# Shamir-Lab/Faucet

Hardware: AMD Instinct MI355X
Metric: canonical k-mers/s (load+scan) at k=31, 100bp reads; % HBM roofline (higher is better)
Workload: dtype u64

## Files before the change

### faucet_amd/csrc/fgpu_ctx.h

```cpp
#pragma once
#include <chrono>
#include <hip/hip_runtime.h>
#include <stdint.h>
#include <stdio.h>
#include <string.h>

#include <string>
#include <thread>
#include <vector>

#include "../../include/faucet_gpu.h"
#include <deque>

#include "fgpu_device.h"

#define FGPU_PADW 8
#define FGPU_USUAL_SPAN (1ULL << 26)
#define FGPU_MAX_SPAN (1ULL << 26)

#define FGPU_RANGE_EVENTS 16
#define FGPU_RANGE_MIN (1ULL << 20)

struct DevBuf {
    void*    p = nullptr;
    uint64_t bytes = 0;
};

struct BatchBufs {
    DevBuf codes, bad;
    DevBuf readflag;
    DevBuf pending;
    DevBuf sure;
    DevBuf fail;
    DevBuf same;
    DevBuf valid, pm, ps, ff, fb, cf0, cf1, cb0, cb1, inF, inB;
    DevBuf lk;
    DevBuf cand;
    uint32_t cand_gen = 0;
    DevBuf nF, nB, need;
    DevBuf kh;
    DevBuf cr;
    DevBuf ps_prefix;
    DevBuf pieces;
    DevBuf sF, sB;
    DevBuf piece_read;
    DevBuf stop_off, stop_out;
    const uint64_t* d_offs = nullptr;
    uint64_t seq = 0;
    bool stops_pending = false;
    uint64_t T = 0;
    uint64_t n_words = 0;
    uint64_t n_reads = 0;
    uint64_t n_pieces = 0;
    uint64_t max_piece_span = 0;
    hipEvent_t pure_done = nullptr;
    hipEvent_t range_ev[FGPU_RANGE_EVENTS] = {};
    uint64_t range_first = 0;
    uint64_t range_span = 0;
    uint64_t n_ranges = 0;
    uint64_t ranges_waited = 0;
    hipEvent_t walk_done = nullptr;
    bool walk_pending = false;
    uint32_t planes_gen = 0;
};

struct ResidentBatch {
    DevBuf codes, bad, sure;
    DevBuf fail;
    DevBuf miss;
    uint64_t T = 0, n_words = 0;
    uint32_t tb = 0;
    void *packed_codes = nullptr, *packed_bad = nullptr;
    const void* codes_p() const { return packed_codes ? packed_codes : codes.p; }
    const void* bad_p() const { return packed_bad ? packed_bad : bad.p; }
    DevBuf offs;
    void* packed_offs = nullptr;
    uint64_t n_reads = 0;
    const void* offs_p() const { return packed_offs ? packed_offs : offs.p; }
};

struct PackedBlock {
    DevBuf buf;
    uint64_t T = 0, n_words = 0, n_reads = 0;
    int state = 0;
    DevBuf offs;
    int offs_state = 0;
    uint64_t resident_index = ~0ULL;
};
static inline uint64_t fgpu_packed_bytes(uint64_t n_words) { return 3 * (n_words + FGPU_PADW) * 8 + 16; }

struct DeltaList {
    DevBuf list, count;
};
#define FGPU_DELTA_RING 4

struct JournalBatch {
    DevBuf codes, bad, offs;
    uint64_t T = 0, n_words = 0, n_reads = 0, seq = 0;
};
#define FGPU_INTERNAL_REPLAY 1000

struct StopBatch {
    uint64_t seq = 0;
    fgpu_stop* data = nullptr;
    size_t n = 0, cap = 0;
};

struct LongPairs {
    int mode = 0;
    bool sparse = false;
    uint64_t tai = 0;
    int n_hash = 0;
    uint32_t* bits = nullptr;
    uint32_t* first = nullptr;
    DevBuf table;
    uint64_t table_high = 0;
    DevBuf canon, h0, h1, vread, rs, state, dev;
    DevBuf kept_set[2];
    int kept_cur = 0;
    uint32_t* flips_host = nullptr;
    bool pending_first = false;
    uint64_t n_kept = 0;
    uint64_t empty_host = 0;
    uint64_t rounds = 0, max_rounds = 0, batches = 0;
    bool open = false, open_odd = false, open_filter = false;
    uint32_t open_elems = 0, open_vreads = 0;
    hipEvent_t ev_open = nullptr;
};

struct WaitSite {
    const char* file;
    int line;
    uint64_t n;
    double ms;
};

struct KernelStat {
    std::string name;
    uint64_t launches = 0;
    double total_ms = 0;
};

struct PendingEvent {
    int stat;
    hipEvent_t a, b;
};

constexpr unsigned FGPU_LATE_CAP = 256;
struct DevCounters {
    unsigned long long kmers;
    unsigned long long to_bloo2;
    unsigned long long segments;
    unsigned long long pieces;
    unsigned long long nb_jcheck;
    unsigned long long nb_no_juncs;
    unsigned long long nb_processed;
    unsigned long long nb_skipped;
    unsigned long long n_junctions;
    unsigned long long table_slots_used;
    unsigned long long followers;
    unsigned long long max_cluster;
    unsigned long long error_flags;
    unsigned long long max_read_len;
    unsigned long long wt_used;
    unsigned long long pad;
    unsigned long long wt_used_b;
    unsigned long long pad2;
    unsigned long long flag_positions;
    unsigned long long piece_positions;
    unsigned long long valid_reused;
    unsigned long long flags_filled;
    unsigned long long walked_pieces;
// ... 390 lines not shown
```

### faucet_amd/csrc/scan_pure.hip

```cpp
#include <algorithm>

#include "fgpu_ctx.h"
#include "fgpu_flags.h"

namespace {

__global__ void __launch_bounds__(256) k_scan_same(const uint64_t* __restrict__ codes, const uint64_t* __restrict__ kept_codes, uint64_t n_code_words,
                                                   const uint64_t* __restrict__ bad, const uint64_t* __restrict__ kept_bad, uint64_t n_words,
                                                   uint32_t* same) {
    bool differ = false;
    for (uint64_t i = (uint64_t)blockIdx.x * blockDim.x + threadIdx.x; i < n_code_words; i += (uint64_t)gridDim.x * blockDim.x) {
        differ |= codes[i] != kept_codes[i];
        if (i < n_words) differ |= bad[i] != kept_bad[i];
    }
    if (__ballot(differ) && fd_lane() == 0) *same = 0;
}

__global__ void __launch_bounds__(256) k_scan_valid(const uint64_t* __restrict__ codes, const uint64_t* __restrict__ bad,
                                                    uint64_t T, uint64_t n_words, FdParams fp, const uint32_t* __restrict__ bloom,
                                                    const uint64_t* __restrict__ sure, const uint32_t* __restrict__ same,
                                                    uint64_t* __restrict__ valid, DevCounters* cnt) {
    unsigned long long n_ok = 0, n_reused = 0;
    const uint64_t total = n_words * 64;
    const bool reuse = sure && *same != 0;
    for (uint64_t p = (uint64_t)blockIdx.x * blockDim.x + threadIdx.x; p < total; p += (uint64_t)gridDim.x * blockDim.x) {
        bool ok = p < T && fd_window_ok(bad, p, fp.k);
        bool v = false;
        if (ok) {
            n_ok++;
            if (reuse && ((sure[p >> 6] >> (p & 63)) & 1ULL)) {
                v = true;
                n_reused++;
            } else {
                v = fd_bloom_contains_canon(bloom, fd_canon(fd_kmer_at(codes, p, fp.k), fp.k), fp.tai_mask, fp.n_hash);
            }
        }
        uint64_t vm = __ballot(v);
        if (fd_lane() == 0) valid[p >> 6] = vm;
    }
    block_add(&cnt->kmers, n_ok);
    block_add(&cnt->valid_reused, n_reused);
}

__global__ void __launch_bounds__(256) k_scan_pieces(const uint64_t* __restrict__ valid, const uint64_t* __restrict__ bad,
                                                     uint64_t n_words, FdParams fp, int check_segment,
                                                     unsigned long long* pm, uint64_t* __restrict__ ps, DevCounters* cnt) {
    unsigned long long n_pieces = 0;
    for (uint64_t w = (uint64_t)blockIdx.x * blockDim.x + threadIdx.x; w < n_words; w += (uint64_t)gridDim.x * blockDim.x) {
        uint64_t vw = valid[w];
        uint64_t prev = w ? valid[w - 1] >> 63 : 0;
        uint64_t starts = vw & ~((vw << 1) | prev);
        uint64_t psw = 0;
        while (starts) {
            const int sbit = __builtin_ctzll(starts);
            starts &= starts - 1;
            const uint64_t p = w * 64 + sbit;
            uint64_t q = p, len = 0;
            for (;;) {
                uint64_t bits = ~fd_bits_at(valid, q);
                if (bits) { len += __builtin_ctzll(bits); break; }
                len += 64;
                q += 64;
            }
            bool piece = len >= (uint64_t)fp.k;
            if (piece && check_segment) {
                uint64_t b = p;
                while (b > 0 && !((bad[(b - 1) >> 6] >> ((b - 1) & 63)) & 1ULL)) b--;
                uint64_t e = p;
                for (;;) {
                    uint64_t bits = fd_bits_at(bad, e);
                    if (bits) { e += __builtin_ctzll(bits); break; }
                    e += 64;
                }
                piece = (e - b) >= (uint64_t)(fp.k + 2 * fp.j + 1);
            }
            if (piece) {
                psw |= 1ULL << sbit;
                n_pieces++;
                uint64_t a = p, z = p + len;
                while (a < z) {
                    uint64_t wi = a >> 6;
                    uint64_t hi = (wi + 1) << 6;
                    uint64_t upto = z < hi ? z : hi;
                    int lo_b = (int)(a & 63), n_b = (int)(upto - a);
                    unsigned long long m = (n_b == 64 ? ~0ULL : ((1ULL << n_b) - 1)) << lo_b;
                    atomicOr(&pm[wi], m);
                    a = upto;
                }
            }
        }
        ps[w] = psw;
    }
    block_add(&cnt->pieces, n_pieces);
}

constexpr int SCAN_BLOCK = 1024;
__global__ void __launch_bounds__(SCAN_BLOCK) k_prefix_block(const uint64_t* __restrict__ ps, uint64_t n_words,
                                                             uint32_t* __restrict__ prefix, uint32_t* __restrict__ block_sums) {
    __shared__ uint32_t sh[SCAN_BLOCK];
    uint64_t w = (uint64_t)blockIdx.x * SCAN_BLOCK + threadIdx.x;
    uint32_t c = w < n_words ? (uint32_t)__popcll(ps[w]) : 0;
    sh[threadIdx.x] = c;
    __syncthreads();
    for (int o = 1; o < SCAN_BLOCK; o <<= 1) {
        uint32_t t = threadIdx.x >= (unsigned)o ? sh[threadIdx.x - o] : 0;
        __syncthreads();
        sh[threadIdx.x] += t;
// ... 348 lines not shown
    out[i] = (signed char)r;
}

}

void fgpu_touch_scan_pure() {
    hipFuncAttributes attr;
    (void)hipFuncGetAttributes(&attr, (const void*)k_scan_same);
}

int fgpu_util_probe_stage3(fgpu_ctx* ctx, const uint64_t* d_kmers, uint64_t n, int mode, signed char* d_out) {
    FGPU_LAUNCH("probe_stage3", k_probe_stage3, fgpu_blocks(n, 256), 256, d_kmers, n, mode, ctx->fd, (const uint32_t*)ctx->bloo2, d_out);
    return FGPU_OK;
}

static int scan_pure_flags(fgpu_ctx* ctx, uint64_t w_lo, uint64_t w_hi) {
    BatchBufs& bb = *ctx->cur;
    const uint64_t nw = w_hi - w_lo;
    const unsigned flags_grid = (unsigned)std::min<uint64_t>(std::max<uint64_t>(nw / 16, 1), 2 * FGPU_GRID_BLOCKS);
    static const int sm_blocks = getenv("FGPU_FLAGS_SM_BLOCKS") ? atoi(getenv("FGPU_FLAGS_SM_BLOCKS")) : 4096;
    if (ctx->fd.j <= 1 && sm_blocks > 0) {
        const unsigned sm_grid = (unsigned)std::min<uint64_t>(std::max<uint64_t>((nw + 255) / 256, 1), (uint64_t)sm_blocks);
        FGPU_LAUNCH("scan_flags", k_scan_flags_sm<1>, sm_grid, 256, (const uint64_t*)bb.codes.p, (const uint64_t*)bb.pm.p,
                    (const uint64_t*)bb.need.p, bb.T, w_lo, w_hi, ctx->fd, (const uint32_t*)ctx->bloo2, (unsigned long long*)bb.ff.p,
                    (unsigned long long*)bb.fb.p, (unsigned long long*)bb.cf0.p, (unsigned long long*)bb.cf1.p,
                    (unsigned long long*)bb.cb0.p, (unsigned long long*)bb.cb1.p, ctx->counters);
    } else
        FGPU_LAUNCH("scan_flags", k_scan_flags, flags_grid, 256, (const uint64_t*)bb.codes.p, (const uint64_t*)bb.pm.p,
                    (const uint64_t*)bb.need.p, bb.T, w_lo, w_hi, ctx->fd, (const uint32_t*)ctx->bloo2, (unsigned long long*)bb.ff.p,
                    (unsigned long long*)bb.fb.p, (unsigned long long*)bb.cf0.p, (unsigned long long*)bb.cf1.p,
                    (unsigned long long*)bb.cb0.p, (unsigned long long*)bb.cb1.p, ctx->counters);
    return FGPU_OK;
}

static void scan_range_plan(const fgpu_ctx* ctx, const BatchBufs& bb, bool one_range, uint64_t* first, uint64_t* further) {
    const uint64_t whole = bb.n_words * 64;
    *first = *further = whole;
    if (one_range || !bb.range_ev[0] || ctx->scan_range_log2 == 0) return;
    if (ctx->scan_range_log2 > 0) { *first = *further = 1ULL << ctx->scan_range_log2; return; }
    const uint64_t span = ctx->window_span;
    if (span >= bb.T || bb.T < 2 * FGPU_RANGE_MIN) return;
    const uint64_t n_windows = (bb.T + span - 1) / span;
    uint64_t m = (uint64_t)(2.0 * (double)bb.T / (3.0 * (double)span) + 0.5);
    m = std::min<uint64_t>(std::max<uint64_t>(m, 1), n_windows - 1);
    const uint64_t cut = (m * span + bb.max_piece_span + 63) & ~63ULL;
    if (cut + FGPU_RANGE_MIN > bb.T) return;
    *first = cut;
    *further = whole - cut;
}

static int scan_pure_back(fgpu_ctx* ctx, bool one_range) {
    BatchBufs& bb = *ctx->cur;
    int rc;
    uint64_t first, further;
    scan_range_plan(ctx, bb, one_range, &first, &further);
    const uint64_t first_words = std::max<uint64_t>(first / 64, 1), further_words = std::max<uint64_t>(further / 64, 1);
    const uint64_t reach_words = (bb.max_piece_span + 63) / 64 + 1;
    bb.range_first = first_words * 64;
    bb.range_span = further_words * 64;
    bb.n_ranges = bb.n_words <= first_words ? 1 : 1 + (bb.n_words - first_words + further_words - 1) / further_words;
    uint64_t looked = 0;
    for (uint64_t r = 0, lo = 0; lo < bb.n_words; r++) {
        const uint64_t hi = std::min(bb.n_words, lo + (r ? further_words : first_words));
        const uint64_t look_to = std::min(bb.n_words, hi + reach_words);
        if (looked < look_to) {
            if ((rc = fgpu_stage_scan_need_lookup(ctx, looked, look_to))) return rc;
            looked = look_to;
        }
        if ((rc = fgpu_stage_scan_need_prewalk(ctx, lo, hi)) || (rc = scan_pure_flags(ctx, lo, hi)) || (rc = fgpu_stage_scan_debug_drop(ctx, lo, hi))) return rc;
        if (bb.n_ranges > 1) FGPU_HIP(hipEventRecord(bb.range_ev[r % FGPU_RANGE_EVENTS], ctx->stream));
        lo = hi;
    }
    return FGPU_OK;
}

int fgpu_stage_scan_pure(fgpu_ctx* ctx, uint64_t* n_pieces, bool one_range) {
    BatchBufs& bb = *ctx->cur;
    *n_pieces = 0;
    bb.n_pieces = 0;
    bb.n_ranges = 0;
    if (bb.T == 0) return FGPU_OK;
    const uint64_t wb = (bb.n_words + FGPU_PADW) * 8;
    int rc;
    DevBuf* planes[] = {&bb.valid, &bb.pm, &bb.ps, &bb.ff, &bb.fb, &bb.cf0, &bb.cf1, &bb.cb0, &bb.cb1, &bb.inF, &bb.inB, &bb.lk, &bb.nF, &bb.nB, &bb.need};
    for (DevBuf* b : planes)
        if ((rc = fgpu_ensure_b(ctx, b, wb))) return rc;
    if ((rc = fgpu_ensure_b(ctx, &bb.ps_prefix, (bb.n_words + FGPU_PADW + bb.n_words / SCAN_BLOCK + 2) * 4))) return rc;
    const double t_a = fgpu_host_now();
    FGPU_HIP(hipMemsetAsync(bb.valid.p, 0, wb, ctx->stream));
    FGPU_HIP(hipMemsetAsync(bb.pm.p, 0, wb, ctx->stream));
    FGPU_HIP(hipMemsetAsync(bb.ps.p, 0, wb, ctx->stream));

    const unsigned grid = fgpu_grid(bb.n_words * 64, 256);
    const unsigned wgrid = fgpu_grid(bb.n_words, 256);
    if ((rc = fgpu_util_count_segments(ctx, ctx->cur->bad.p, ctx->cur->n_words, ctx->fd.k + 2 * ctx->fd.j + 1))) return rc;
    const uint64_t kept_index = ctx->scan_resident_base + ctx->scan_batch_index;
    const ResidentBatch* kept = kept_index < ctx->resident_count ? ctx->resident[kept_index] : nullptr;
    ctx->scan_batch_index++;
    if (kept && (kept->T != bb.T || kept->n_words != bb.n_words)) kept = nullptr;
    const bool taken = ctx->scan_take_kept != nullptr;
    if (taken) kept = ctx->scan_take_kept;
    if (kept) {
        if ((rc = fgpu_ensure_b(ctx, &bb.same, 64))) return rc;
        FGPU_HIP(hipMemsetAsync(bb.same.p, 0x01, 4, ctx->stream));
        const uint64_t ncw = 2 * bb.n_words;
        if (!taken)
            FGPU_LAUNCH("scan_same", k_scan_same, fgpu_grid(ncw, 256), 256, (const uint64_t*)bb.codes.p, (const uint64_t*)kept->codes_p(), ncw,
                        (const uint64_t*)bb.bad.p, (const uint64_t*)kept->bad_p(), bb.n_words, (uint32_t*)bb.same.p);
    }
    FGPU_LAUNCH("scan_valid", k_scan_valid, grid, 256, (const uint64_t*)bb.codes.p, (const uint64_t*)bb.bad.p, bb.T, bb.n_words, ctx->fd,
                (const uint32_t*)ctx->bloo2, kept ? (const uint64_t*)kept->sure.p : (const uint64_t*)nullptr,
                kept ? (const uint32_t*)bb.same.p : (const uint32_t*)nullptr, (uint64_t*)bb.valid.p, ctx->counters);
    const int check_segment = ctx->fd.k < 2 * ctx->fd.j + 2;
    FGPU_LAUNCH("scan_pieces", k_scan_pieces, wgrid, 256, (const uint64_t*)bb.valid.p, (const uint64_t*)bb.bad.p, bb.n_words, ctx->fd,
                check_segment, (unsigned long long*)bb.pm.p, (uint64_t*)bb.ps.p, ctx->counters);
    uint32_t* prefix = (uint32_t*)bb.ps_prefix.p;
    uint32_t* block_sums = prefix + bb.n_words + FGPU_PADW;
    const uint32_t nblk = fgpu_blocks(bb.n_words + 1, SCAN_BLOCK);
    const uint64_t nw1 = bb.n_words + 1;
    FGPU_LAUNCH("prefix_block", k_prefix_block, nblk, SCAN_BLOCK, (const uint64_t*)bb.ps.p, nw1, prefix, block_sums);
    FGPU_LAUNCH("prefix_sums", k_prefix_sums, 1, SCAN_BLOCK, block_sums, nblk);
    FGPU_LAUNCH("prefix_apply", k_prefix_apply, fgpu_blocks(nw1, 256), 256, prefix, (const uint32_t*)block_sums, nw1);
    FGPU_HIP(hipMemcpyAsync(ctx->counters_host, ctx->counters, sizeof(DevCounters), hipMemcpyDeviceToHost, ctx->stream));
    const double t_b = fgpu_host_now();
    FGPU_HIP(fgpu_sync_stream(ctx, ctx->stream));
    const double t_c = fgpu_host_now();
    ctx->host_ms[2] += t_b - t_a;
    ctx->host_ms[3] += t_c - t_b;
    bb.max_piece_span = ctx->counters_host->max_read_len + 64;
    const uint64_t np = ctx->counters_host->pieces - ctx->scan_pieces_seen;
    ctx->scan_pieces_seen = ctx->counters_host->pieces;
    *n_pieces = np;
    bb.n_pieces = np;
    if ((rc = fgpu_ensure_b(ctx, &bb.pieces, (np + 1) * sizeof(uint2)))) return rc;
    if (np) {
        FGPU_LAUNCH("piece_list", k_scan_piece_list, wgrid, 256, (const uint64_t*)bb.ps.p, (const uint64_t*)bb.pm.p,
                    (const uint32_t*)prefix, bb.n_words, (uint2*)bb.pieces.p);
        if (ctx->record_stops) {
            if ((rc = fgpu_ensure_b(ctx, &bb.piece_read, np * 4))) return rc;
            FGPU_LAUNCH("piece_read", k_scan_piece_read, fgpu_blocks(np, 256), 256, (const uint2*)bb.pieces.p, np, bb.d_offs, bb.n_reads,
                        (uint32_t*)bb.piece_read.p);
        }
        if ((rc = fgpu_stage_scan_need(ctx))) return rc;
        DevBuf* outs[] = {&bb.ff, &bb.fb, &bb.cf0, &bb.cf1, &bb.cb0, &bb.cb1};
        for (DevBuf* o : outs) FGPU_HIP(hipMemsetAsync(o->p, 0, wb, ctx->stream));
        if ((rc = scan_pure_back(ctx, one_range))) return rc;
    }
    ctx->host_ms[4] += fgpu_host_now() - t_c;
    return FGPU_OK;
}
```

### faucet_amd/csrc/scan_walk.hip

```cpp
#include <cstring>
#include <algorithm>

#include "fgpu_flags.h"
#include "walk_tables.h"

namespace {

__device__ __forceinline__ uint32_t uf_find(uint32_t* parent, uint32_t x) {
    uint32_t p = ld_agent(&parent[x]);
    while (p != x) {
        uint32_t gp = ld_agent(&parent[p]);
        if (gp != p) atomicMin(&parent[x], gp);
        x = p;
        p = gp;
    }
    return x;
}

__device__ __forceinline__ void uf_union(uint32_t* parent, uint32_t a, uint32_t b) {
    for (;;) {
        a = uf_find(parent, a);
        b = uf_find(parent, b);
        if (a == b) return;
        if (a < b) { uint32_t t = a; a = b; b = t; }
// ... 2049 lines not shown
__global__ void __launch_bounds__(256) k_delta_filter_add(const uint32_t* __restrict__ list, const unsigned long long* __restrict__ count, uint32_t* dfilter,
                                                          uint64_t dmask) {
    const uint64_t n = *count;
    for (uint64_t i = (uint64_t)blockIdx.x * blockDim.x + threadIdx.x; i < n; i += (uint64_t)gridDim.x * blockDim.x) {
        const uint32_t h32 = list[i];
        atomicOr(&dfilter[delta_word(h32, dmask)], delta_bits(h32));
    }
}

}

void fgpu_touch_scan_walk() {
    hipFuncAttributes attr;
    (void)hipFuncGetAttributes(&attr, (const void*)k_iota_u32);
}

int fgpu_scan_alloc(fgpu_ctx* ctx) {
    if (ctx->jkeys) return FGPU_OK;
    ctx->jcap = ctx->prm.junction_capacity;
    if (const char* e = getenv("FGPU_WALK_KO")) ctx->walk_ko = (uint32_t)std::max(0, atoi(e));
    ctx->walk_ko_always = getenv("FGPU_WALK_KO_ALWAYS") != nullptr || (ctx->prm.flags & FGPU_FLAG_KEY_ORDER_FROM_START) != 0;
    if ((ctx->prm.flags & FGPU_FLAG_KEY_ORDER_FROM_START) && !getenv("FGPU_WALK_KO")) ctx->walk_ko = 32;
    ctx->walk_ko_weight = (ctx->prm.flags & FGPU_FLAG_KEY_ORDER_FROM_START) ? 128u : 0u;
    if (const char* e = getenv("FGPU_WALK_KO_WEIGHT")) ctx->walk_ko_weight = (uint32_t)std::max(0, atoi(e));
    if (const char* e = getenv("FGPU_OVW_EV_LOG2")) ctx->ovw_ev_log2 = std::min(27, std::max(8, atoi(e)));
    if (const char* e = getenv("FGPU_OVW_ROUNDS")) ctx->ovw_rounds = std::max(0, atoi(e));
    ctx->ko_hk_cap = 1u << 22;
    ctx->ko_occ_cap = 1u << 24;
    {
        size_t free_b = 0, total_b = 0;
        if (hipMemGetInfo(&free_b, &total_b) == hipSuccess)
            while (ctx->max_span > FGPU_MAX_SPAN && 40ULL * ctx->max_span > free_b / 4) ctx->max_span >>= 1;
        (void)hipGetLastError();
    }
    for (;;) {
        while (ctx->max_span / (uint64_t)(ctx->fd.k + 1) + 2 >= W_OWNER_MASK) ctx->max_span >>= 1;
        ctx->wcap = 4 * ctx->max_span;
        ctx->wmax = (uint32_t)(ctx->max_span / (uint64_t)(ctx->fd.k + 1) + 2);
        struct { void** p; uint64_t bytes; } want[] = {
            {(void**)&ctx->jkeys, ctx->jcap * 8}, {(void**)&ctx->jrecs, ctx->jcap * 32}, {(void**)&ctx->jstamps, ctx->jcap * 16}, {(void**)&ctx->jfilter, ctx->jcap * 2 / 8},
            {(void**)&ctx->wdesc, 64}, {(void**)&ctx->wkeys, ctx->wcap * 8},
            {(void**)&ctx->wbits, 2 * (1ULL << ctx->wbits_log2) / 8},
            {(void**)&ctx->uf_parent, 2ULL * ctx->wmax * 4},
            {(void**)&ctx->cl_count, 2ULL * ctx->wmax * 4}, {(void**)&ctx->cl_offset, 2ULL * ctx->wmax * 4}, {(void**)&ctx->cl_fill, (uint64_t)ctx->wmax * 4},
            {(void**)&ctx->cl_weight, 2ULL * ctx->wmax * 4}, {(void**)&ctx->ko_hk, (uint64_t)ctx->ko_hk_cap * 4 * 3},
            {(void**)&ctx->ko_occ, (uint64_t)ctx->ko_occ_cap * (4 * 3 + 8)}, {(void**)&ctx->ko_piece, (uint64_t)ctx->wmax * 4 * 2 + 64},
            {(void**)&ctx->cl_members, (uint64_t)ctx->wmax * 4 * 2}, {(void**)&ctx->cl_roots, (uint64_t)ctx->wmax * 4 + 64}};
        hipError_t err = hipSuccess;
        uint64_t failed_bytes = 0;
        for (auto& w : want) {
            *w.p = nullptr;
            if ((err = hipMalloc(w.p, w.bytes)) != hipSuccess) { *w.p = nullptr; failed_bytes = w.bytes; break; }
        }
        if (err == hipSuccess) return FGPU_OK;
        (void)hipGetLastError();
        for (auto& w : want) { if (*w.p) hipFree(*w.p); *w.p = nullptr; }
        if (ctx->max_span <= FGPU_MAX_SPAN) {
            ctx->err = std::string("the scan's tables do not fit the device (hipMalloc of ") + std::to_string(failed_bytes) + " bytes: " + hipGetErrorString(err) + ")";
            return FGPU_ERR_NOMEM;
        }
        ctx->max_span >>= 1;
    }
}

int fgpu_scan_reset(fgpu_ctx* ctx) {
    if (int rc = fgpu_scan_clear_table(ctx)) return rc;
    if (!ctx->wt_epoch) FGPU_HIP(hipMemsetAsync(ctx->wkeys, 0, ctx->wcap * 8, ctx->stream));
    FGPU_HIP(hipMemsetAsync(ctx->wbits, 0, 2 * (1ULL << ctx->wbits_log2) / 8, ctx->stream));
    FGPU_LAUNCH("iota", k_iota_u32, 64, 256, ctx->uf_parent, (uint64_t)ctx->wmax);
    FGPU_LAUNCH("iota", k_iota_u32, 64, 256, ctx->uf_parent + ctx->wmax, (uint64_t)ctx->wmax);
    FGPU_HIP(hipMemsetAsync(ctx->cl_count, 0, 2 * ctx->wmax * 4, ctx->stream));
    FGPU_HIP(hipMemsetAsync(ctx->cl_offset, 0xFF, 2 * ctx->wmax * 4, ctx->stream));
    FGPU_HIP(hipMemsetAsync(ctx->cl_weight, 0, 2 * ctx->wmax * 4, ctx->stream));
    FGPU_HIP(hipMemsetAsync(ctx->ko_hk, 0xFF, (size_t)ctx->ko_hk_cap * 4 * 2, ctx->stream));
    FGPU_HIP(hipMemsetAsync(ctx->ko_hk + 2 * (size_t)ctx->ko_hk_cap, 0, (size_t)ctx->ko_hk_cap * 4, ctx->stream));
    FGPU_HIP(hipMemsetAsync(ctx->ko_piece, 0, (size_t)ctx->wmax * 4 * 2 + 64, ctx->stream));
    return FGPU_OK;
}

int fgpu_stage_scan_need(fgpu_ctx* ctx) {
    BatchBufs& bb = *ctx->cur;
    const uint64_t wb = (bb.n_words + FGPU_PADW) * 8;
    const bool eager = (ctx->prm.flags & FGPU_FLAG_EAGER_FLAGS) || ctx->eager_runtime || ctx->eager_scan;
    FGPU_HIP(hipMemsetAsync(bb.need.p, eager ? 0xFF : 0, wb, ctx->stream));
    if (!bb.n_pieces) return FGPU_OK;
    return fgpu_ensure_b(ctx, &bb.kh, (bb.n_words + FGPU_PADW) * 64 * 4);
}

int fgpu_stage_scan_need_lookup(fgpu_ctx* ctx, uint64_t w_lo, uint64_t w_hi) {
    BatchBufs& bb = *ctx->cur;
    if (!bb.n_pieces || w_lo >= w_hi) return FGPU_OK;
    FGPU_LAUNCH("need_lookup", k_need_lookup, fgpu_grid((w_hi - w_lo) * 64, 256), 256, (const uint64_t*)bb.codes.p, (const uint64_t*)bb.pm.p,
                w_hi, ctx->fd, make_jt(ctx), (uint64_t*)bb.nF.p, (uint64_t*)bb.nB.p, (uint32_t*)bb.kh.p, w_lo);
    return FGPU_OK;
}

int fgpu_stage_scan_need_prewalk(fgpu_ctx* ctx, uint64_t w_lo, uint64_t w_hi) {
    BatchBufs& bb = *ctx->cur;
    const bool eager = (ctx->prm.flags & FGPU_FLAG_EAGER_FLAGS) || ctx->eager_runtime || ctx->eager_scan;
    if (eager || !bb.n_pieces || w_lo >= w_hi) return FGPU_OK;
    static const int need_tight = getenv("FGPU_NEED_TIGHT") ? atoi(getenv("FGPU_NEED_TIGHT")) : 2;
    const uint64_t most = std::min<uint64_t>(bb.n_pieces, (w_hi - w_lo) * 64 / (uint64_t)(ctx->fd.k + 1) + 2);
    FGPU_LAUNCH("need_prewalk", k_need_prewalk, fgpu_grid(most, 256), 256, (const uint64_t*)bb.codes.p, (const uint2*)bb.pieces.p,
                (const uint32_t*)bb.ps_prefix.p, w_lo, w_hi, ctx->fd, make_jt(ctx), (const uint64_t*)bb.nF.p, (const uint64_t*)bb.nB.p,
                (unsigned long long*)bb.need.p, need_tight);
    return FGPU_OK;
}

int fgpu_scan_refresh_planes(fgpu_ctx* ctx, BatchBufs* b) {
    if (!b->n_pieces || !b->T) return FGPU_OK;
    JTable jt = make_jt(ctx);
    ctx->launch_stream = ctx->stream;
    FGPU_LAUNCH("need_lookup", k_refresh_lookup, fgpu_grid(b->n_words * 64, 256), 256, (const uint64_t*)b->codes.p, (const uint64_t*)b->pm.p, b->n_words,
                ctx->fd, jt, (const uint32_t*)jt.filter, jt.filter_mask, (uint64_t*)b->nF.p, (uint64_t*)b->nB.p, (const uint32_t*)b->kh.p, 0, (uint64_t*)nullptr);
    if (b->pure_done) FGPU_HIP(hipEventRecord(b->pure_done, ctx->stream));
    return FGPU_OK;
}

int fgpu_scan_build_cand(fgpu_ctx* ctx, BatchBufs* b) {
    b->cand_gen = 0;
    if (!b->n_pieces || !b->T) return FGPU_OK;
    int rc;
    const uint64_t wb = (b->n_words + FGPU_PADW) * 8;
    if ((rc = fgpu_ensure_b(ctx, &b->cand, wb)) || (rc = fgpu_ensure(ctx, &ctx->cand_filter, (1ULL << CAND_FILTER_LOG2) / 8))) return rc;
    ctx->launch_stream = ctx->stream;
    FGPU_HIP(hipMemsetAsync(ctx->cand_filter.p, 0, (1ULL << CAND_FILTER_LOG2) / 8, ctx->stream));
    FGPU_HIP(hipMemsetAsync(b->cand.p, 0, wb, ctx->stream));
    const unsigned word_blocks = std::min(fgpu_blocks(b->n_words, 256), 2048u), piece_blocks = std::min(fgpu_blocks(b->n_pieces, 256), 2048u);
    FGPU_LAUNCH("cand_plane", k_cand_mark, word_blocks + piece_blocks, 256, (const uint64_t*)b->pm.p, (const uint64_t*)b->nF.p, (const uint64_t*)b->nB.p,
                (const uint64_t*)b->ff.p, (const uint64_t*)b->fb.p, (const uint32_t*)b->kh.p, b->n_words, (const uint2*)b->pieces.p, b->n_pieces, ctx->fd,
                (uint32_t*)ctx->cand_filter.p, word_blocks);
    FGPU_LAUNCH("cand_plane", k_cand_probe, fgpu_grid(b->n_words * 64, 256), 256, (const uint64_t*)b->pm.p, (const uint32_t*)b->kh.p, b->n_words,
                (const uint32_t*)ctx->cand_filter.p, (uint64_t*)b->cand.p);
    if (b->pure_done) FGPU_HIP(hipEventRecord(b->pure_done, ctx->stream));
    b->cand_gen = ctx->hint_gen;
    return FGPU_OK;
}

int fgpu_stage_scan_debug_drop(fgpu_ctx* ctx, uint64_t w_lo, uint64_t w_hi) {
    static const int drop = getenv("FGPU_DEBUG_NEED_DROP") ? atoi(getenv("FGPU_DEBUG_NEED_DROP")) : 0;
    BatchBufs& bb = *ctx->cur;
    if (!drop || !bb.n_pieces || w_lo >= w_hi) return FGPU_OK;
    if (drop == 2 && ((ctx->prm.flags & FGPU_FLAG_EAGER_FLAGS) || ctx->eager_runtime || ctx->eager_scan)) return FGPU_OK;
    FGPU_LAUNCH("debug_need_drop", k_debug_need_drop, fgpu_grid(w_hi - w_lo, 256), 256, w_lo, w_hi, (uint64_t*)bb.ff.p, (uint64_t*)bb.fb.p,
                (uint64_t*)bb.need.p, (uint64_t*)bb.cf0.p, (uint64_t*)bb.cf1.p, (uint64_t*)bb.cb0.p, (uint64_t*)bb.cb1.p, drop,
                (const uint64_t*)bb.pm.p, (const uint32_t*)bb.kh.p);
    return FGPU_OK;
}

static int env_int(const char* name, int absent) { const char* e = getenv(name); return e ? atoi(e) : absent; }
static bool env_is_one(const char* name) { const char* e = getenv(name); return e && e[0] == '1'; }
struct WalkKnobs {
    const bool no_overlap = env_is_one("FGPU_NO_OVERLAP");
    const unsigned cluster_grid = (unsigned)std::max(1, env_int("FGPU_CLUSTER_GRID", 256));
    const uint64_t refresh_div = (uint64_t)std::max(1, env_int("FGPU_REFRESH_DIV", 4));
    const unsigned delta_per_block = (unsigned)std::max(1, env_int("FGPU_DELTA_PER_BLOCK", 1024));
    const int ko_avg = getenv("FGPU_WALK_KO_AVG") ? std::min(255, std::max(0, env_int("FGPU_WALK_KO_AVG", 0))) : -1;
    const int ko_avg_min = getenv("FGPU_WALK_KO_AVG_MIN") ? std::min(255, std::max(1, env_int("FGPU_WALK_KO_AVG_MIN", 0))) : -1;
    const int ovw_followers = env_int("FGPU_OVW_FOLLOWERS", 0);
    const unsigned walk_dyn_grid = (unsigned)std::max(1, env_int("FGPU_WALK_DYN_GRID", 1024));
    const bool dbg_span = getenv("FGPU_DEBUG_SPAN") != nullptr;
};
static const WalkKnobs& walk_knobs() { static const WalkKnobs knobs; return knobs; }
bool fgpu_walk_no_overlap() { return walk_knobs().no_overlap; }

struct WalkBatch {
    BatchBufs& bb;
// ... 275 lines not shown
                wb.seq_base, kt, ot, rule.ovw_rounds, ctx->counters, kn.ovw_followers, (const unsigned long long*)evb, (uint64_t)1 << ev_log2, epoch_first);
    if (wb.ovw_stream != wb.walk_stream) {
        FGPU_HIP(hipEventRecord(ctx->ev_settled, wb.ovw_stream));
        ctx->launch_stream = wb.walk_stream;
    }
    return FGPU_OK;
}

static int walk_clusters(fgpu_ctx* ctx, const WalkKnobs& kn, const WalkBatch& wb, const WalkWindow& w, const LargeClusterRule& rule, const KoTables& kt,
                         const OvwTables& ot) {
    const unsigned walk_grid_w = fgpu_blocks(w.max_pieces, 64);
    const unsigned ko_grid = 512;
    const uint32_t ko_ticket = 64;
    FGPU_LAUNCH("walk", k_walk_dyn, std::min(walk_grid_w, kn.walk_dyn_grid), 64, wb.pl, ctx->fd, wb.jt, (const uint32_t*)w.root_list, w.roots_state,
                (const uint32_t*)w.cl_count, (const uint32_t*)w.cl_offset, (const uint32_t*)ctx->cl_members, ctx->cl_members + ctx->wmax, (const WinDesc*)ctx->wdesc,
                wb.seq_base, (const uint32_t*)ctx->bloo2, ctx->counters, (const uint32_t*)w.cl_weight, (const uint32_t*)kt.bad,
                (const uint32_t*)kt.state, rule.ko_heavy, (uint32_t)ctx->scan_windows, rule.ko_heavy_w);
    if (rule.ovw_on && wb.ovw_stream != wb.walk_stream) FGPU_HIP(hipStreamWaitEvent(wb.walk_stream, ctx->ev_settled, 0));
    if (rule.ko_heavy) {
        FGPU_LAUNCH("walk_ko_prepare", k_ko_rank, 256, 256, kt, (const uint32_t*)ot.state, rule.ovw_rounds);
        FGPU_LAUNCH("walk_ko", k_walk_ko, ko_grid, 64, wb.pl, ctx->fd, wb.jt, (const uint32_t*)ctx->cl_fill, (const uint32_t*)w.cl_count, (const WinDesc*)ctx->wdesc,
                    wb.seq_base, (const uint32_t*)ctx->bloo2, ctx->counters, kt, rule.ko_heavy, ko_ticket, (const uint32_t*)w.cl_weight, rule.ko_heavy_w,
                    (const uint32_t*)ot.state, (const uint32_t*)ot.longp, rule.ovw_rounds);
    }
    return FGPU_OK;
}

static int walk_collect_and_reset(fgpu_ctx* ctx, const WalkBatch& wb, const WalkWindow& w) {
    const BatchBufs& bb = wb.bb;
    const uint64_t w_first = w.lo >> 6, w_last = std::min<uint64_t>(bb.n_words, (w.pos_end + 63) / 64);
    FGPU_LAUNCH("walk_delta", k_delta_collect, (unsigned)std::min<uint64_t>(fgpu_blocks(w_last - w_first, 256), 256), 256, (unsigned long long*)bb.cr.p,
                (const uint32_t*)bb.kh.p, w_first, w_last, (uint32_t*)wb.created->list.p, (unsigned long long*)wb.created->count.p, wb.pl,
                (const WinDesc*)ctx->wdesc, ctx->counters, (uint32_t)ctx->scan_windows);
    FGPU_HIP(hipEventRecord(ctx->ev_walked, wb.walk_stream));
    FGPU_HIP(hipStreamWaitEvent(ctx->cstream, ctx->ev_walked, 0));
    ctx->launch_stream = ctx->cstream;
    FGPU_LAUNCH("walk_clean", k_walk_reset_uf, std::min(256u, fgpu_blocks(w.max_pieces, 256)), 256, w.uf_parent, w.cl_count, w.cl_offset, w.cl_weight, (uint32_t)w.max_pieces,
                (uint4*)w.wt.bits, (uint32_t)((1u << ctx->wbits_log2) / 128));
    ctx->launch_stream = wb.walk_stream;
    FGPU_HIP(hipEventRecord(ctx->ev_uf_reset[w.parity], ctx->cstream));
    return FGPU_OK;
}

static int walk_span_look(fgpu_ctx* ctx, const WalkKnobs& kn, hipStream_t walk_stream, uint64_t* span_now) {
    if (ctx->calib_left <= 0 || ctx->prm.walk_window_span) return FGPU_OK;
    FGPU_HIP(hipMemcpyAsync(ctx->fb_host, &ctx->counters->followers, 8, hipMemcpyDeviceToHost, walk_stream));
    FGPU_HIP(hipMemcpyAsync(ctx->fb_host + 1, &ctx->counters->walked_pieces, 8, hipMemcpyDeviceToHost, walk_stream));
    FGPU_HIP(hipMemcpyAsync(ctx->fb_host + 2, &ctx->counters->ko_overflows, 8, hipMemcpyDeviceToHost, walk_stream));
    FGPU_HIP(fgpu_sync_stream(ctx, walk_stream));
    uint64_t span = *span_now;
    const uint64_t f = ctx->fb_host[0] - ctx->calib_f, p = ctx->fb_host[1] - ctx->calib_p;
    if (ctx->fb_host[2] > ctx->calib_ovf && span > 4096) {
        ctx->calib_ovf = ctx->fb_host[2];
        ctx->calib_f = ctx->fb_host[0];
        ctx->calib_p = ctx->fb_host[1];
        span = std::max<uint64_t>(4096, span / 4);
        ctx->proven_span = std::min(ctx->proven_span, span);
        ctx->calib_left = std::max(ctx->calib_left, 4);
        ctx->span_ceiling = std::min(ctx->span_ceiling, span * 2);
        if (kn.dbg_span) fprintf(stderr, "[span] look: the large-cluster walks' tables overflowed -> span %llu, looks left %d\n", (unsigned long long)span, ctx->calib_left);
    } else if (p >= 64) {
        ctx->calib_f = ctx->fb_host[0];
        ctx->calib_p = ctx->fb_host[1];
        bool shrunk = false;
        const uint64_t ceiling = std::min<uint64_t>(ctx->max_span, ctx->span_ceiling), usual = std::min<uint64_t>(ceiling, FGPU_USUAL_SPAN);
        if (f * 2 > p && span > 4096) { span /= 2; shrunk = true; }
        else if (f * 3 < p && span < usual) span = std::min<uint64_t>(span * 4, usual);
        else if (f * 16 < p && span < ceiling) span = std::min<uint64_t>(span * 4, ceiling);
        else ctx->calib_left = 1;
        ctx->calib_left--;
        if (!shrunk && span >= (1ULL << 22)) ctx->calib_left = 0;
        if (kn.dbg_span) fprintf(stderr, "[span] look: followers %llu of %llu pieces -> span %llu, looks left %d\n", (unsigned long long)f, (unsigned long long)p,
                                 (unsigned long long)span, ctx->calib_left);
    }
    *span_now = span;
    return FGPU_OK;
}

int fgpu_stage_scan_walk(fgpu_ctx* ctx, uint64_t n_pieces) {
    if (!n_pieces) return FGPU_OK;
    const WalkKnobs& kn = walk_knobs();
    BatchBufs& bb = *ctx->cur;
    int rc;
    const uint64_t wbytes = (bb.n_words + FGPU_PADW) * 8;
    Planes pl{(const uint64_t*)bb.codes.p, (const uint64_t*)bb.pm.p, (const uint64_t*)bb.ps.p, (const uint32_t*)bb.ps_prefix.p,
              (const uint64_t*)bb.ff.p, (const uint64_t*)bb.fb.p, (const uint64_t*)bb.cf0.p, (const uint64_t*)bb.cf1.p,
              (const uint64_t*)bb.cb0.p, (const uint64_t*)bb.cb1.p, (uint64_t*)bb.nF.p, (uint64_t*)bb.nB.p, (const uint2*)bb.pieces.p,
              (uint64_t*)bb.lk.p, (const uint64_t*)bb.need.p, nullptr, nullptr, (const uint32_t*)bb.kh.p, nullptr};
    if ((rc = fgpu_ensure_b(ctx, &bb.cr, wbytes))) return rc;
    pl.cr = (unsigned long long*)bb.cr.p;
    if (ctx->record_stops) {
        if ((rc = fgpu_ensure_b(ctx, &bb.sF, wbytes)) || (rc = fgpu_ensure_b(ctx, &bb.sB, wbytes))) return rc;
        pl.sF = (unsigned long long*)bb.sF.p;
        pl.sB = (unsigned long long*)bb.sB.p;
    }
    const uint64_t span = ctx->window_span;
    const uint64_t ext = bb.max_piece_span;
    if (ctx->max_span + ext + 64 > ctx->wcap) {
        ctx->err = "a read of " + std::to_string(ext) + " bases is longer than the walk's window tables allow";
        return FGPU_ERR_CAPACITY;
    }
    if (ext >= (1ULL << (STAMP_SHIFT - 1)) - 64) {
        ctx->err = "a read of " + std::to_string(ext) + " bases is longer than the junction creation stamps allow (2^19 windows)";
        return FGPU_ERR_CAPACITY;
    }
    hipStream_t walk_stream = kn.no_overlap ? ctx->stream : ctx->wstream;
    hipStream_t ovw_stream = (!kn.no_overlap && ctx->ostream) ? ctx->ostream : walk_stream;
    WalkBatch wb{bb, pl, make_jt(ctx), bb.T, ext, ctx->scan_piece_base, walk_stream, ovw_stream, false, &ctx->delta_ring[ctx->delta_next % FGPU_DELTA_RING]};
    const uint64_t T = wb.T;
    ctx->launch_stream = walk_stream;
    bb.ranges_waited = 0;
    if (bb.n_ranges <= 1 && bb.pure_done) FGPU_HIP(hipStreamWaitEvent(walk_stream, bb.pure_done, 0));
    if (ctx->dbg_stall_us) FGPU_LAUNCH("debug_stall", k_debug_stall, 1, 1, (unsigned long long)ctx->dbg_stall_us * 100ULL);
    if (ctx->refresh_snapshot && (rc = walk_refresh_prepared(ctx, bb, wb.jt, walk_stream, &wb.cand_ok))) return rc;
    if (ctx->record_stops) {
        FGPU_HIP(hipMemsetAsync(bb.sF.p, 0, wbytes, walk_stream));
        FGPU_HIP(hipMemsetAsync(bb.sB.p, 0, wbytes, walk_stream));
    }
    FGPU_HIP(hipMemsetAsync(bb.cr.p, 0, wbytes, walk_stream));
    {
        const uint64_t now = ctx->counters_host->n_junctions;
        ctx->delta_hist[ctx->delta_next % FGPU_DELTA_RING] = now;
        const uint64_t back = ctx->delta_next >= (uint64_t)(FGPU_DELTA_RING - 1) ? ctx->delta_hist[(ctx->delta_next - (FGPU_DELTA_RING - 1)) % FGPU_DELTA_RING] : 0;
        ctx->delta_ring_keys = now > back ? now - back : 0;
        ctx->delta_batch_base = now;
    }
    if ((rc = fgpu_ensure_b(ctx, &wb.created->list, (bb.n_words + FGPU_PADW) * 64 * 4)) || (rc = fgpu_ensure(ctx, &wb.created->count, 64))) return rc;
    FGPU_HIP(hipMemsetAsync(wb.created->count.p, 0, 8, walk_stream));
    const int stage_tok = fgpu_prof_begin(ctx, "walk_stage");
    ctx->prof_suppress = !ctx->prof_walk_detail;
    uint64_t span_now = span;
    const bool whole_batch = wb.cand_ok && !ctx->prm.walk_window_span && ctx->calib_left <= 0 && span * 2 >= T && span < T && T <= ctx->max_span &&
                             bb.n_pieces <= ctx->wmax;
    for (uint64_t lo = 0, step = 0; lo < T; lo += step) {
        step = whole_batch ? T : span_now;
        WalkWindow w;
        KoTables kt;
        OvwTables ot;
        if ((rc = walk_window_begin(ctx, wb, lo, std::min<uint64_t>(T, lo + step), &w))) return rc;
        if ((rc = walk_register(ctx, kn, wb, w)) || (rc = walk_link(ctx, wb, w))) return rc;
        const LargeClusterRule rule = large_cluster_rule(ctx, kn);
        FGPU_LAUNCH("walk_cluster", k_walk_cluster, std::min(kn.cluster_grid, fgpu_blocks(w.max_pieces, 256)), 256, (const uint32_t*)w.uf_parent, w.cl_count, w.cl_offset,
                    ctx->cl_fill, ctx->cl_members, pl, lo, w.hi, (WinDesc*)ctx->wdesc, ctx->counters, w.cl_weight, rule.ko_heavy_w, w.root_list, w.roots_state);
        if ((rc = walk_large_tables(ctx, wb, rule, kt, ot)) || (rc = walk_large_first(ctx, kn, wb, w, rule, kt, ot)) || (rc = walk_clusters(ctx, kn, wb, w, rule, kt, ot)) ||
            (rc = walk_collect_and_reset(ctx, wb, w)))
            return rc;
        ctx->scan_windows++;
        if ((rc = walk_span_look(ctx, kn, walk_stream, &span_now))) return rc;
    }
    if (ctx->delta_ready)
        FGPU_LAUNCH("walk_delta", k_delta_filter_add, 256, 256, (const uint32_t*)wb.created->list.p, (const unsigned long long*)wb.created->count.p,
                    (uint32_t*)ctx->delta_filter.p, ctx->delta_filter_bits - 1);
    ctx->delta_next++;
    ctx->window_span = span_now;
    ctx->prof_suppress = false;
    fgpu_prof_end(ctx, stage_tok);
    if (bb.walk_done) {
        FGPU_HIP(hipEventRecord(bb.walk_done, walk_stream));
        bb.walk_pending = true;
    }
    ctx->launch_stream = ctx->stream;
    ctx->scan_piece_base += n_pieces;
    return FGPU_OK;
}
```

Before: 6.108 billion.

## Pack zero-initialized scan planes into one arena cleared by a single memset

Moves the per-batch planes that must start at zero (valid, pm, ps, need, flag planes, cr, sF/sB) plus the 'same' flag into one contiguous arena. One hipMemsetAsync then clears it, replacing about a dozen separate memsets spread across the scan and walk stages. The 'same' flag meaning is inverted (0 now means identical) so the zeroed arena header gives the right default without its own memset. The walk-stream memsets of cr/sF/sB move to the main stream earlier, which changes cross-stream ordering and assumes those buffers are not still in use by a previous batch's walk.

Result: no change. 6.049 billion (-1.0%).

```diff
diff --git a/faucet_amd/csrc/fgpu_ctx.h b/faucet_amd/csrc/fgpu_ctx.h
--- a/faucet_amd/csrc/fgpu_ctx.h
+++ b/faucet_amd/csrc/fgpu_ctx.h
@@ -32,6 +32,7 @@
     DevBuf pending;
     DevBuf sure;
     DevBuf fail;
+    DevBuf arena;
     DevBuf same;
     DevBuf valid, pm, ps, ff, fb, cf0, cf1, cb0, cb1, inF, inB;
     DevBuf lk;
@@ -88,6 +89,9 @@
     uint64_t resident_index = ~0ULL;
 };
 static inline uint64_t fgpu_packed_bytes(uint64_t n_words) { return 3 * (n_words + FGPU_PADW) * 8 + 16; }
+
+#define FGPU_ARENA_HEADER 256
+static inline uint64_t fgpu_arena_stride(uint64_t n_words) { return ((n_words + FGPU_PADW) * 8 + 255) & ~255ULL; }
 
 struct DeltaList {
     DevBuf list, count;
diff --git a/faucet_amd/csrc/scan_pure.hip b/faucet_amd/csrc/scan_pure.hip
--- a/faucet_amd/csrc/scan_pure.hip
+++ b/faucet_amd/csrc/scan_pure.hip
@@ -13,7 +13,7 @@
         differ |= codes[i] != kept_codes[i];
         if (i < n_words) differ |= bad[i] != kept_bad[i];
     }
-    if (__ballot(differ) && fd_lane() == 0) *same = 0;
+    if (__ballot(differ) && fd_lane() == 0) *same = 1;
 }
 
 __global__ void __launch_bounds__(256) k_scan_valid(const uint64_t* __restrict__ codes, const uint64_t* __restrict__ bad,
@@ -22,7 +22,7 @@
                                                     uint64_t* __restrict__ valid, DevCounters* cnt) {
     unsigned long long n_ok = 0, n_reused = 0;
     const uint64_t total = n_words * 64;
-    const bool reuse = sure && *same != 0;
+    const bool reuse = sure && *same == 0;
     for (uint64_t p = (uint64_t)blockIdx.x * blockDim.x + threadIdx.x; p < total; p += (uint64_t)gridDim.x * blockDim.x) {
         bool ok = p < T && fd_window_ok(bad, p, fp.k);
         bool v = false;
@@ -537,14 +537,19 @@
     if (bb.T == 0) return FGPU_OK;
     const uint64_t wb = (bb.n_words + FGPU_PADW) * 8;
     int rc;
-    DevBuf* planes[] = {&bb.valid, &bb.pm, &bb.ps, &bb.ff, &bb.fb, &bb.cf0, &bb.cf1, &bb.cb0, &bb.cb1, &bb.inF, &bb.inB, &bb.lk, &bb.nF, &bb.nB, &bb.need};
+    DevBuf* planes[] = {&bb.inF, &bb.inB, &bb.lk, &bb.nF, &bb.nB};
     for (DevBuf* b : planes)
         if ((rc = fgpu_ensure_b(ctx, b, wb))) return rc;
     if ((rc = fgpu_ensure_b(ctx, &bb.ps_prefix, (bb.n_words + FGPU_PADW + bb.n_words / SCAN_BLOCK + 2) * 4))) return rc;
+    DevBuf* zeroed[] = {&bb.valid, &bb.pm, &bb.ps, &bb.need, &bb.ff, &bb.fb, &bb.cf0, &bb.cf1, &bb.cb0, &bb.cb1, &bb.cr, &bb.sF, &bb.sB};
+    const uint64_t n_zeroed = ctx->record_stops ? 13 : 11;
+    const uint64_t stride = fgpu_arena_stride(bb.n_words), arena_bytes = FGPU_ARENA_HEADER + n_zeroed * stride;
+    if ((rc = fgpu_ensure_b(ctx, &bb.arena, arena_bytes))) return rc;
+    bb.same = DevBuf{bb.arena.p, FGPU_ARENA_HEADER};
+    for (uint64_t i = 0; i < 13; i++)
+        *zeroed[i] = i < n_zeroed ? DevBuf{(char*)bb.arena.p + FGPU_ARENA_HEADER + i * stride, stride} : DevBuf{};
     const double t_a = fgpu_host_now();
-    FGPU_HIP(hipMemsetAsync(bb.valid.p, 0, wb, ctx->stream));
-    FGPU_HIP(hipMemsetAsync(bb.pm.p, 0, wb, ctx->stream));
-    FGPU_HIP(hipMemsetAsync(bb.ps.p, 0, wb, ctx->stream));
+    FGPU_HIP(hipMemsetAsync(bb.arena.p, 0, arena_bytes, ctx->stream));
 
     const unsigned grid = fgpu_grid(bb.n_words * 64, 256);
     const unsigned wgrid = fgpu_grid(bb.n_words, 256);
@@ -556,8 +561,6 @@
     const bool taken = ctx->scan_take_kept != nullptr;
     if (taken) kept = ctx->scan_take_kept;
     if (kept) {
-        if ((rc = fgpu_ensure_b(ctx, &bb.same, 64))) return rc;
-        FGPU_HIP(hipMemsetAsync(bb.same.p, 0x01, 4, ctx->stream));
         const uint64_t ncw = 2 * bb.n_words;
         if (!taken)
             FGPU_LAUNCH("scan_same", k_scan_same, fgpu_grid(ncw, 256), 256, (const uint64_t*)bb.codes.p, (const uint64_t*)kept->codes_p(), ncw,
@@ -597,8 +600,6 @@
                         (uint32_t*)bb.piece_read.p);
         }
         if ((rc = fgpu_stage_scan_need(ctx))) return rc;
-        DevBuf* outs[] = {&bb.ff, &bb.fb, &bb.cf0, &bb.cf1, &bb.cb0, &bb.cb1};
-        for (DevBuf* o : outs) FGPU_HIP(hipMemsetAsync(o->p, 0, wb, ctx->stream));
         if ((rc = scan_pure_back(ctx, one_range))) return rc;
     }
     ctx->host_ms[4] += fgpu_host_now() - t_c;
diff --git a/faucet_amd/csrc/scan_walk.hip b/faucet_amd/csrc/scan_walk.hip
--- a/faucet_amd/csrc/scan_walk.hip
+++ b/faucet_amd/csrc/scan_walk.hip
@@ -2155,7 +2155,7 @@
     BatchBufs& bb = *ctx->cur;
     const uint64_t wb = (bb.n_words + FGPU_PADW) * 8;
     const bool eager = (ctx->prm.flags & FGPU_FLAG_EAGER_FLAGS) || ctx->eager_runtime || ctx->eager_scan;
-    FGPU_HIP(hipMemsetAsync(bb.need.p, eager ? 0xFF : 0, wb, ctx->stream));
+    if (eager) FGPU_HIP(hipMemsetAsync(bb.need.p, 0xFF, wb, ctx->stream));
     if (!bb.n_pieces) return FGPU_OK;
     return fgpu_ensure_b(ctx, &bb.kh, (bb.n_words + FGPU_PADW) * 64 * 4);
 }
@@ -2597,15 +2597,12 @@
     const WalkKnobs& kn = walk_knobs();
     BatchBufs& bb = *ctx->cur;
     int rc;
-    const uint64_t wbytes = (bb.n_words + FGPU_PADW) * 8;
     Planes pl{(const uint64_t*)bb.codes.p, (const uint64_t*)bb.pm.p, (const uint64_t*)bb.ps.p, (const uint32_t*)bb.ps_prefix.p,
               (const uint64_t*)bb.ff.p, (const uint64_t*)bb.fb.p, (const uint64_t*)bb.cf0.p, (const uint64_t*)bb.cf1.p,
               (const uint64_t*)bb.cb0.p, (const uint64_t*)bb.cb1.p, (uint64_t*)bb.nF.p, (uint64_t*)bb.nB.p, (const uint2*)bb.pieces.p,
               (uint64_t*)bb.lk.p, (const uint64_t*)bb.need.p, nullptr, nullptr, (const uint32_t*)bb.kh.p, nullptr};
-    if ((rc = fgpu_ensure_b(ctx, &bb.cr, wbytes))) return rc;
     pl.cr = (unsigned long long*)bb.cr.p;
     if (ctx->record_stops) {
-        if ((rc = fgpu_ensure_b(ctx, &bb.sF, wbytes)) || (rc = fgpu_ensure_b(ctx, &bb.sB, wbytes))) return rc;
         pl.sF = (unsigned long long*)bb.sF.p;
         pl.sB = (unsigned long long*)bb.sB.p;
     }
@@ -2628,11 +2625,6 @@
     if (bb.n_ranges <= 1 && bb.pure_done) FGPU_HIP(hipStreamWaitEvent(walk_stream, bb.pure_done, 0));
     if (ctx->dbg_stall_us) FGPU_LAUNCH("debug_stall", k_debug_stall, 1, 1, (unsigned long long)ctx->dbg_stall_us * 100ULL);
     if (ctx->refresh_snapshot && (rc = walk_refresh_prepared(ctx, bb, wb.jt, walk_stream, &wb.cand_ok))) return rc;
-    if (ctx->record_stops) {
-        FGPU_HIP(hipMemsetAsync(bb.sF.p, 0, wbytes, walk_stream));
-        FGPU_HIP(hipMemsetAsync(bb.sB.p, 0, wbytes, walk_stream));
-    }
-    FGPU_HIP(hipMemsetAsync(bb.cr.p, 0, wbytes, walk_stream));
     {
         const uint64_t now = ctx->counters_host->n_junctions;
         ctx->delta_hist[ctx->delta_next % FGPU_DELTA_RING] = now;
```
